# syoyo/lucille

Measured on AMD Instinct MI355X. Metric: Mrays/s (primary+AO), higher is better.
Workload: dtype f32 filter + f64 resolve (hit records f64); 1 GPU; S-soup-1M ray dump (BASELINE config 3): 1000000 random triangles, one dump of 100000000 incoherent rays cut into 1 contiguous slice(s), closest-hit; rays=100000000, rays_per_gpu=100000000, triangles=1000000, mode=closest, variant=-1, parallelism=replicated BVH, ray slices x1

## Files before the change

### include/lucille_hip.h

```cpp
#ifndef LUCILLE_HIP_H
#define LUCILLE_HIP_H

#include <stddef.h>
#include <stdint.h>

#ifdef __cplusplus
extern "C" {
#endif

#define LH_MISS      0xFFFFFFFFu
#define LH_INFINITY  1.0e38

#define LH_MODE_CLOSEST 0
#define LH_MODE_ANY     1

#define LH_VARIANT_DEFAULT (-1)

typedef struct lh_accel lh_accel_t;
typedef struct lh_rib_scene lh_rib_scene_t;

typedef struct lh_accel_info {
    uint32_t ntriangles;
    uint32_t nnodes;
    uint32_t nleaves;
// ... 78 lines not shown

int  lh_accel_intersect_device_tmax(lh_accel_t *accel, size_t n_rays, const void *d_org_xyz, const void *d_dir_xyz,
                                    const void *d_tmax, int ray_format, int record_format,
                                    void *d_prim_or_rec16, void *d_t, void *d_u, void *d_v, void *d_occluded, int mode,
                                    const void *d_index, size_t n_index, const void *d_count, void *stream);
int  lh_accel_intersect_host_tmax(lh_accel_t *accel, size_t n, const void *org_xyz, const void *dir_xyz, const void *tmax,
                                  int ray_format, int record_format, void *prim_or_rec16, double *t, double *u, double *v,
                                  uint8_t *occluded, int mode);

int  lh_accel_intersect_device_counted(lh_accel_t *accel, size_t n, const void *d_org_xyz,
                                       const void *d_dir_xyz, void *d_prim, void *d_t,
                                       void *d_u, void *d_v, void *d_occluded, int mode,
                                       int variant, uint64_t counters[4]);
uint64_t lh_accel_last_retraced(const lh_accel_t *accel);
int lh_accel_dump_node_bytes(const lh_accel_t *accel);

int  lh_accel_trace_statistics(lh_accel_t *accel, int enable);
int  lh_accel_statistics(lh_accel_t *accel, uint64_t counters[5], int clear);
int  lh_accel_slot_statistics(lh_accel_t *accel, uint64_t slots[3], int clear);

int  lh_accel_set_grid(lh_accel_t *accel, int blocks);
int  lh_accel_set_param(lh_accel_t *accel, const char *name, int value);


typedef struct lh_camera {
    int    width, height;
    int    rh;
    int    ortho;
    double flength;
    double cam2world[16];
// ... 215 lines not shown
```

### lucille_amd/binding.py

```python
import atexit
import ctypes as C
import os
import subprocess
import weakref

import numpy as np

HERE = os.path.dirname(os.path.abspath(__file__))
CSRC = os.path.join(HERE, "csrc")

MISS = 0xFFFFFFFF
T_INF = 1.0e38
MODE_CLOSEST, MODE_ANY = 0, 1
VARIANT_DEFAULT, VARIANT_DIRECT, VARIANT_SPEC = -1, 0, 4
RAYS_F64, RAYS_F32 = 0, 1
REC_F64, REC16 = 0, 1
SELECT_HIT, SELECT_MISS, SELECT_OCCLUDED, SELECT_UNOCCLUDED = 0, 1, 2, 3
POS_F64, POS_F32 = 0, 1
AO_NO_HIT = 0xFFFFFFFF


class LucilleHipError(RuntimeError):
    pass

# ... 66 lines not shown


class DirtParams(C.Structure):
    _fields_ = [("near_clip", C.c_double), ("far_clip", C.c_double), ("eps", C.c_double)]

    def __init__(self, near_clip=0.1, far_clip=0.5, eps=1.0e-5):
        super().__init__(float(near_clip), float(far_clip), float(eps))


BEAM_SET_DTYPE = np.dtype([("org", np.float64, (3,)), ("dir", np.float64, (4, 3)), ("normal", np.float64, (4, 3)),
                           ("dominant_axis", np.int32), ("dirsign", np.int32, (3,))])

ABI_SYMBOLS = [
    "lh_device_count", "lh_last_error", "lh_accel_create", "lh_accel_add_mesh", "lh_accel_add_mesh_device", "lh_accel_commit", "lh_accel_wait_exact", "lh_accel_ref_tree",
    "lh_accel_destroy", "lh_accel_info", "lh_accel_prim_lookup", "lh_accel_intersect1", "lh_accel_combine_statistics", "lh_accel_intersect_diag_host", "lh_accel_intersect_diag_device",
    "lh_accel_intersect_host", "lh_accel_intersect_device", "lh_accel_intersect_host_ex", "lh_accel_intersect_device_ex", "lh_accel_intersect_device_indexed", "lh_accel_intersect_device_tmax", "lh_accel_intersect_host_tmax", "lh_accel_compact_device", "lh_accel_intersect_device_counted", "lh_accel_last_retraced", "lh_accel_dump_node_bytes",
    "lh_accel_set_grid", "lh_accel_set_param", "lh_accel_export", "lh_accel_set_normals", "lh_render_primary_rays",
    "lh_render_ao_tile", "lh_render_ao_tile_host", "lh_render_ao_bands", "lh_render_scratch", "lh_accel_beam_visibility_host", "lh_accel_beam_visibility_device", "lh_accel_beam_visibility_set_host", "lh_accel_beam_raster_host", "lh_accel_beam_raster_device", "lh_accel_beam_raster_set_host", "lh_render_pt_tile",
    "lh_accel_trace_statistics", "lh_accel_statistics", "lh_accel_slot_statistics",
    "lh_render_ao_frame_host", "lh_rib_load", "lh_rib_free", "lh_rib_last_error", "lh_rib_info", "lh_rib_messages",
    "lh_rib_mesh", "lh_accel_add_rib_scene", "lh_hdr_write",
    "lh_accel_set_material", "lh_accel_set_environment", "lh_render_pt_tile2", "lh_render_pt_bands", "lh_accel_set_attribute", "lh_accel_set_normals_device", "lh_accel_set_attribute_device",
    "lh_accel_state_build_device", "lh_accel_state_build_host", "lh_accel_ao_device", "lh_accel_ao_host", "lh_accel_ao_rays_device",
    "lh_accel_dirt_device", "lh_accel_dirt_host", "lh_render_dirt_tile",
    "lh_multi_create", "lh_multi_destroy", "lh_multi_ndevices", "lh_multi_accel", "lh_multi_add_mesh", "lh_multi_set_normals",
    "lh_multi_add_rib_scene", "lh_multi_commit", "lh_multi_set_material", "lh_multi_set_environment", "lh_multi_intersect_host",
    "lh_multi_render_ao_frame_host", "lh_multi_render_pt_frame_host",
    "lh_synth_soup_triangles", "lh_synth_soup_rays", "lh_synth_tessellate", "lh_synth_skip",
    "lh_dist_unique_id", "lh_dist_init", "lh_dist_init_file", "lh_dist_destroy", "lh_dist_rank", "lh_dist_world", "lh_dist_transport",
    "lh_dist_barrier", "lh_dist_host_barrier", "lh_dist_broadcast", "lh_dist_gather", "lh_dist_pack_records16", "lh_dist_broadcast_scene", "lh_dist_render_ao_frame_host",
]
# ... 28 lines not shown
    L.lh_accel_destroy.restype = None
    L.lh_accel_info.argtypes = [vp, C.POINTER(AccelInfo)]
    L.lh_accel_prim_lookup.argtypes = [vp, u32, C.POINTER(u32), C.POINTER(u32)]
    L.lh_accel_intersect1.argtypes = [vp, vp, vp, C.POINTER(u32), C.POINTER(C.c_double),
                                      C.POINTER(C.c_double), C.POINTER(C.c_double)]
    L.lh_accel_intersect_host.argtypes = [vp, sz, vp, vp, vp, vp, vp, vp, vp, i32]
    L.lh_accel_intersect_device.argtypes = [vp, sz, vp, vp, vp, vp, vp, vp, vp, i32, i32, vp]
    L.lh_accel_intersect_host_ex.argtypes = [vp, sz, vp, vp, i32, i32, vp, vp, vp, vp, vp, i32]
    L.lh_accel_intersect_device_ex.argtypes = [vp, sz, vp, vp, i32, i32, vp, vp, vp, vp, vp, i32, vp]
    L.lh_accel_intersect_device_indexed.argtypes = [vp, sz, vp, vp, i32, i32, vp, vp, vp, vp, vp, i32, vp, sz, vp, vp]
    L.lh_accel_compact_device.argtypes = [sz, i32, vp, vp, i32, vp, sz, vp, vp, vp, vp]
    L.lh_accel_intersect_device_tmax.argtypes = [vp, sz, vp, vp, vp, i32, i32, vp, vp, vp, vp, vp, i32, vp, sz, vp, vp]
    L.lh_accel_intersect_host_tmax.argtypes = [vp, sz, vp, vp, vp, i32, i32, vp, vp, vp, vp, vp, i32]
    L.lh_accel_last_retraced.argtypes = [vp]; L.lh_accel_last_retraced.restype = C.c_uint64
    L.lh_accel_dump_node_bytes.argtypes = [vp]
    L.lh_accel_intersect_device_counted.argtypes = [vp, sz, vp, vp, vp, vp, vp, vp, vp, i32, i32,
                                                    C.POINTER(C.c_uint64)]
    L.lh_accel_set_grid.argtypes = [vp, i32]
    L.lh_accel_set_param.argtypes = [vp, C.c_char_p, i32]
    L.lh_accel_trace_statistics.argtypes = [vp, i32]
    L.lh_accel_statistics.argtypes = [vp, C.POINTER(C.c_uint64), i32]
    L.lh_accel_slot_statistics.argtypes = [vp, C.POINTER(C.c_uint64), i32]
    L.lh_accel_export.argtypes = [vp, vp, vp]
    L.lh_accel_set_normals.argtypes = [vp, u32, vp, sz, i32]
    L.lh_accel_set_normals_device.argtypes = [vp, u32, u32, vp, i32, sz, i32, vp]
    L.lh_accel_set_attribute_device.argtypes = [vp, u32, i32, u32, vp, i32, sz, vp]
    L.lh_render_primary_rays.argtypes = [vp, C.POINTER(Camera), i32, i32, i32, i32, i32, vp, vp, vp]
    L.lh_render_ao_tile.argtypes = [vp, C.POINTER(Camera), i32, i32, i32, i32, i32, i32, C.c_uint64, vp, vp,
                                    C.POINTER(TileStats), vp]
    L.lh_render_ao_bands.argtypes = [vp, C.POINTER(Camera), i32, C.POINTER(i32), i32, i32, i32, C.c_uint64, vp, C.POINTER(TileStats), vp]
# ... 425 lines not shown
        return out

    def trace_statistics(self, enable=True):
        _check(self.L.lh_accel_trace_statistics(self.h, 1 if enable else 0), "lh_accel_trace_statistics")

    def statistics(self, clear=False):
        c = (C.c_uint64 * 5)()
        _check(self.L.lh_accel_statistics(self.h, c, 1 if clear else 0), "lh_accel_statistics")
        return dict(zip(("nodes", "tris", "exact", "rays", "hits"), (int(x) for x in c)))

    def slot_statistics(self, clear=False):
        c = (C.c_uint64 * 3)()
        _check(self.L.lh_accel_slot_statistics(self.h, c, 1 if clear else 0), "lh_accel_slot_statistics")
        return dict(zip(("node_slots", "tri_slots", "regroups"), (int(x) for x in c)))

    def dump_node_bytes(self):
        return int(self.L.lh_accel_dump_node_bytes(self.h))

    def beam_raster(self, org, corner_dirs, corners, width, height, frame, eye, fov, t_init=None):
        o = np.ascontiguousarray(org, np.float64).reshape(-1, 3); n = o.shape[0]
        d = np.ascontiguousarray(corner_dirs, np.float64).reshape(n, 4, 3)
        c = np.ascontiguousarray(corners, np.float64).reshape(n, 3)
        pl = RasterPlane(int(width), int(height), (C.c_double * 9)(*np.asarray(frame, np.float64).reshape(-1)),
                         (C.c_double * 3)(*np.asarray(eye, np.float64).reshape(-1)), float(fov))
        t = np.zeros((n, height, width)) if t_init is None else np.ascontiguousarray(t_init, np.float64).reshape(n, height, width).copy()
        st = np.empty(n, np.int32); fl = np.zeros((n, 4), np.uint64)
        _check(self.L.lh_accel_beam_raster_host(self.h, n, o.ctypes.data, d.ctypes.data, c.ctypes.data, C.addressof(pl),
                                                t.ctypes.data, st.ctypes.data, fl.ctypes.data), "lh_accel_beam_raster_host")
        return t, st, fl

# ... 475 lines not shown
```

### lucille_amd/csrc/lh_commit.hip

```cpp
#include <assert.h>
#include <thread>
#include <vector>

#include "lh_internal.h"
#include "lh_danger.h"

static thread_local char g_err[512] = "";

extern "C" void lh_set_error(const char *msg) { snprintf(g_err, sizeof(g_err), "%s", msg ? msg : ""); }

int lh_fail(const char *fmt, ...)
{
    va_list ap; va_start(ap, fmt); vsnprintf(g_err, sizeof(g_err), fmt, ap); va_end(ap);
    return -1;
}

pthread_mutex_t g_scene_mu = PTHREAD_MUTEX_INITIALIZER;

extern "C" const char *lh_last_error(void) { return g_err; }

extern "C" int lh_device_count(void)
{
    int n = 0;
    if (hipGetDeviceCount(&n) != hipSuccess) return 0;
// ... 34 lines not shown
    if (env && atoi(env) > 0 && atoi(env) <= 64) { a->tri_batch = atoi(env); a->knobs_user = 1; }
    env = getenv("LH_MIN_ACTIVE");
    if (env && atoi(env) > 0 && atoi(env) <= 64) { a->min_active = atoi(env); a->knobs_user = 1; }
    a->ray_chunk = 256;
    env = getenv("LH_RAY_CHUNK");
    if (env && atoi(env) > 0 && atoi(env) <= (1 << 20)) a->ray_chunk = (uint32_t)atoi(env);
    a->dev.ray_chunk = a->ray_chunk;
    a->dev.ray_budget = LH_RAY_BUDGET; a->dump_budget = LH_DUMP_BUDGET;
    a->ao_budget = LH_AO_BUDGET;
    env = getenv("LH_AO_BUDGET");
    if (env && atoi(env) > 0) { a->ao_budget = (uint32_t)atoi(env); a->ao_budget_user = 1; }
    env = getenv("LH_DUMP_BUDGET");
    if (env && atoi(env) > 0) a->dump_budget = (uint32_t)atoi(env);
    env = getenv("LH_RAY_BUDGET");
    if (env && atoi(env) > 0) a->dev.ray_budget = (uint32_t)atoi(env);
    a->dev.top_nodes = LH_TOP_AUTO;
    a->dev.deg_dcap = INFINITY; a->dev.cap_srcs = 0u; a->dev.ndanger = LH_DANGER_ALL;
    a->dev.coop_patience = 0;
    a->dev.ao_group = 0;
    env = getenv("LH_AO_GROUP");
    if (env && atoi(env) >= 0 && atoi(env) <= 4096) a->dev.ao_group = (uint32_t)atoi(env);
    env = getenv("LH_TOP_NODES");
    if (env && atoi(env) >= 0 && atoi(env) <= (int)LH_TOP_NODES_MAX) a->dev.top_nodes = (uint32_t)atoi(env);
    *out = a;
    return 0;
}

extern "C" int lh_accel_add_mesh(lh_accel_t *a, uint32_t npos, const double *pos, size_t stride,
                                 uint32_t nidx, const uint32_t *idx)
{
// ... 403 lines not shown
    a->d_prim_mesh = a->d_materials = a->d_env_map = NULL;
    free_buf(&a->r_state); free_buf(&a->r_uni); free_buf(&a->r_bands); free_buf(&a->r_diag);
    if (a->h_read) { (void)hipHostFree(a->h_read); a->h_read = NULL; }
    a->d_total = NULL;
    if (a->d_danger) (void)hipFree(a->d_danger);
    a->d_danger = NULL; a->dev.ndanger = LH_DANGER_ALL;
    if (a->d_cursor) (void)hipFree(a->d_cursor);
    if (a->d_counters) (void)hipFree(a->d_counters);
    for (int k = 0; k < LH_AOQ_SLOTS; k++) {
        lh_fixq_t *q = &a->aoq[k].q;
        if (q->queue) {
            (void)hipFree(q->queue); (void)hipFree(q->qcount);
            (void)hipStreamDestroy((hipStream_t)q->aux_stream); (void)hipEventDestroy((hipEvent_t)q->ev_ready); (void)hipEventDestroy((hipEvent_t)q->ev_done);
        }
        memset(q, 0, sizeof(*q)); a->aoq[k].used = 0;
    }
    if (a->pipe.ready) {
        for (int b = 0; b < a->pipe.depth; b++) {
            (void)hipHostFree(a->pipe.h_in[b]); (void)hipHostFree(a->pipe.h_out[b]);
            (void)hipFree(a->pipe.d_in[b]); (void)hipFree(a->pipe.d_out[b]);
            (void)hipEventDestroy(a->pipe.in_done[b]); (void)hipEventDestroy(a->pipe.done[b]);
        }
        for (int b = 0; b < 3; b++) (void)hipStreamDestroy(a->pipe.s[b]);
        a->pipe.ready = 0;
    }
    if (a->d_stage) (void)hipFree(a->d_stage);
    if (a->stream) (void)hipStreamDestroy(a->stream);
    a->d_cursor = a->d_counters = NULL;
    a->d_stage = NULL; a->stage_bytes = 0; a->stream = NULL;
}
// ... 650 lines not shown
    else if (!strcmp(name, "min_active") && value > 0 && value <= 64) { a->min_active = value; a->knobs_user = 1; }
    else if (!strcmp(name, "tri_batch") && value > 0 && value <= 64) { a->tri_batch = value; a->knobs_user = 1; }
    else if (!strcmp(name, "ray_chunk") && value > 0 && value <= (1 << 20)) { a->ray_chunk = (uint32_t)value; a->dev.ray_chunk = (uint32_t)value; }
    else if (!strcmp(name, "variant") && (value == LH_VARIANT_DIRECT || value == LH_VARIANT_SPEC)) a->default_variant = value;
    else if (!strcmp(name, "ray_budget") && value > 0) { a->dev.ray_budget = (uint32_t)value; a->dump_budget = (uint32_t)value; a->ao_budget = (uint32_t)value; a->ao_budget_user = 1; }
    else if (!strcmp(name, "dump_budget") && value > 0) a->dump_budget = (uint32_t)value;
    else if (!strcmp(name, "ao_budget") && value >= 0) { a->ao_budget = (uint32_t)value; a->ao_budget_user = 1; }
    else if (!strcmp(name, "coop_patience") && value >= 0) a->dev.coop_patience = (uint32_t)value;
    else if (!strcmp(name, "ao_fused")) a->ao_fused = value != 0;
    else if (!strcmp(name, "combine")) a->combine = value != 0;
    else if (!strcmp(name, "host_walk")) { a->host_walk = value != 0; a->hw_gpu_left = 0; a->hw_ns = 0.0; }
    else if (!strcmp(name, "ao_group") && value >= 0 && value <= 4096) a->dev.ao_group = (uint32_t)value;
    else if (!strcmp(name, "fast_start")) a->fast_start = value != 0;
    else if (!strcmp(name, "wide8") && value >= -1 && value <= 1) a->wide8 = value;
    else if (!strcmp(name, "top_nodes") && value >= -1 && value <= (int)LH_TOP_NODES_MAX) a->dev.top_nodes = value < 0 ? LH_TOP_AUTO : (uint32_t)value;
    else if (!strcmp(name, "stack_cap") && (value == 0 || (value >= 8 && value <= 64 && value % 2 == 0))) a->dev.stack_cap = (uint32_t)value;
    else return fail("lh_accel_set_param: unknown parameter or bad value: %s = %d", name, value);
    return 0;
}

extern "C" int lh_accel_export(const lh_accel_t *a, void *nodes, void *tri32)
{
    if (!a || !a->committed) return fail("lh_accel_export: accel not committed");
    if (a->hs->device_meshes) return fail("lh_accel_export: the scene was committed from device meshes; there is no host copy");
    if (a->hs->device_built) return fail("lh_accel_export: the tree was built on the device; there is no host copy");
    if (nodes && a->hs->bvh.nnodes) memcpy(nodes, a->hs->bvh.nodes, sizeof(lh_node_t) * (size_t)a->hs->bvh.nnodes);
    if (tri32 && a->hs->bvh.ntris) memcpy(tri32, a->hs->bvh.tri32, sizeof(lh_tri32_t) * (size_t)a->hs->bvh.ntris);
    return 0;
}

// ... 93 lines not shown
```

### lucille_amd/csrc/lh_internal.h

```cpp
#ifndef LH_INTERNAL_H
#define LH_INTERNAL_H

#include <hip/hip_runtime.h>

#include <math.h>
#include <pthread.h>
#include <stdarg.h>
#include <stdio.h>
#include <stdlib.h>
#include <string.h>
#include <time.h>
#include <unistd.h>

#include "../../include/lucille_hip.h"
#include "lh_bvh.h"
#include "lh_refbvh.h"
#include "lh_device.h"

int lh_fail(const char *fmt, ...);
#define fail lh_fail
#define HIPCHK(x) do { hipError_t e_ = (x); if (e_ != hipSuccess) \
    return lh_fail("%s failed: %s", #x, hipGetErrorString(e_)); } while (0)

struct lh_mesh_copy { uint32_t npos, nidx; double *pos; uint32_t *idx; double *nrm; int two_side;
                      double *attr[5]; };

struct lh_dmesh_attr { void *block; size_t stride; int fmt, has; };
#define LH_DATTR_NORMAL 5
#define LH_DATTR_SLOTS 6
struct lh_dmesh { void *block; const void *pos; const uint32_t *idx; size_t stride; uint32_t npos, ntris; int fmt;
                  uint32_t nidx; int two_side; lh_dmesh_attr attr[LH_DATTR_SLOTS]; };
typedef struct lh_dmesh_desc { const void *pos; const uint32_t *idx; unsigned long long stride; uint32_t npos, fmt; } lh_dmesh_desc_t;
// ... 45 lines not shown
    unsigned cursor_next;
    pthread_mutex_t mu;
    int stat_on;
    unsigned long long stat[5];
    unsigned long long stat_slots[3];
    hipStream_t stream;
    uint64_t device_bytes;
    double upload_seconds;
    int grid_blocks;
    int grid_user;
    int min_active;
    uint32_t ray_chunk;
    int tri_batch;
    int knobs_user;
    int default_variant;
    struct { hipStream_t stream; int used; lh_fixq_t q; } aoq[LH_AOQ_SLOTS];
    void *d_stage; size_t stage_bytes;
    struct { void *h_in[LH_PIPE_DEPTH_MAX], *h_out[LH_PIPE_DEPTH_MAX], *d_in[LH_PIPE_DEPTH_MAX], *d_out[LH_PIPE_DEPTH_MAX]; hipStream_t s[3];
             hipEvent_t in_done[LH_PIPE_DEPTH_MAX], done[LH_PIPE_DEPTH_MAX]; size_t cap; int depth, ready; } pipe;
    void *d_nrm9;
    void *d_attr9[3], *d_st6, *d_inside;
    void *d_prim_mesh;
    lh_material_t *materials; uint32_t nmaterials; void *d_materials; int materials_dirty;
    lh_environment_t env; void *d_env_map; int env_set;
    lh_buf r_state;
    lh_buf r_uni;
    lh_buf r_diag;
    lh_buf r_bands;
    void *h_read;
    lh_buf r_org, r_dir, r_prim, r_t, r_u, r_v, r_frame;
    lh_ao_scratch tile_ao;
    lh_ao_scratch batch_ao;
    lh_buf b_tot, b_host;
    lh_ao_scratch tile_dirt, batch_dirt;
    lh_dirt_scratch tile_dirt_t, batch_dirt_t;
    lh_buf d_tot, d_rays;
    uint64_t last_retraced;
    int ao_fused;
    uint32_t ao_budget;
    int ao_budget_user;
    uint32_t dump_budget;
    int build_auto;
    int poison_outputs;
    int fast_start;
    lh_buf p_org2, p_dir2, p_path, p_path2, p_thr, p_thr2, p_rad, p_counts;
    unsigned long long *d_total;
    size_t r_nsamples, r_nslots, r_nao;
    struct lh_combiner *comb;
    int combine;
    int host_walk; unsigned long long hw_calls; double hw_ns; int hw_gpu_left;
};

#define LH_NCURSOR 64

struct lh_guard {
    pthread_mutex_t *m;
// ... 43 lines not shown
struct lh_launch_opt {
    uint32_t io_fmt = 0u;
    uint32_t *diag_out = NULL;
    const uint32_t *n_dev = NULL;
    const void *cam_src = NULL;
    unsigned long long *diag_clock = NULL;
    bool indexed = false; const uint32_t *index = NULL; uint32_t idx_nrays = 0u;
    const void *tmax = NULL;
};
int  lh_launch(lh_accel_t *a, const lh_batch_t &batch, int variant, hipStream_t s, bool dump, const lh_launch_opt &opt = lh_launch_opt());
static inline unsigned long long *lh_next_cursor(lh_accel_t *a)
{
    return (unsigned long long *)((uint32_t *)a->d_cursor + (size_t)LH_CURSOR_WORDS * (a->cursor_next++ % LH_NCURSOR));
}
int  lh_aoq_slot(lh_accel_t *a, hipStream_t s);
static inline void lh_stat_add(lh_accel_t *a, const unsigned long long *h, unsigned long long rays, unsigned long long hits, bool slots = false)
{
    a->stat[0] += h[LH_CNT_NODES]; a->stat[1] += h[LH_CNT_TRIS]; a->stat[2] += h[LH_CNT_EXACT];
    a->stat[3] += rays; a->stat[4] += hits;
    if (slots) { a->stat_slots[0] += h[LH_CNT_NODE_SLOTS]; a->stat_slots[1] += h[LH_CNT_TRI_SLOTS]; a->stat_slots[2] += h[LH_CNT_REGROUP_SLOTS]; }
}
int  lh_ensure_stage(lh_accel_t *a, size_t bytes);

extern "C" int lh_render_launch_primary(const lh_camera_t *cam, int x0, int y0, int w, int h, int xs, int ys,
                                        double *d_org, double *d_dir, void *stream);
extern "C" int lh_render_launch_compact(const lh_dev_scene_t *sc, const double *d_nrm9, size_t n, const double *d_org,
                                        const double *d_dir, const uint32_t *d_prim, const double *d_t,
                                        const double *d_u, const double *d_v, uint32_t *d_block_counts,
                                        uint32_t *d_slot_of_sample, double *d_hitrec,
                                        unsigned long long *d_slot_key, int x0, int w, int nbands, int band_rows,
// ... 50 lines not shown
```

### lucille_amd/csrc/lh_query.hip

```cpp
#include <atomic>
#include <chrono>
#include <condition_variable>
#include <deque>
#include <mutex>
#include <thread>
#include <vector>

#include "lh_internal.h"

__global__ void k_fill_listed(size_t n, const uint32_t *index, const uint32_t *count, uint32_t nrays, int miss,
                              uint32_t *prim, double *t, double *u, double *v, uint8_t *occ, uint4 *rec16, unsigned long long *counters)
{
    const size_t k = (size_t)blockIdx.x * blockDim.x + threadIdx.x;
    if (count && *count < n) n = *count;
    if (k >= n) return;
    const uint32_t i = index ? index[k] : (uint32_t)k;
    if (i >= nrays) return;
    const uint32_t w = miss ? LH_MISS_PRIM : 0x77777777u;
    const unsigned long long d = 0x7777777777777777ull;
    if (rec16) { uint4 r; r.x = w; r.y = miss ? __float_as_uint((float)LH_T_INF) : w; r.z = r.w = miss ? __float_as_uint(0.0f) : w; rec16[i] = r; }
    if (prim) prim[i] = w;
    if (t) t[i] = miss ? LH_T_INF : __longlong_as_double((long long)d);
    if (u) u[i] = miss ? 0.0 : __longlong_as_double((long long)d);
    if (v) v[i] = miss ? 0.0 : __longlong_as_double((long long)d);
// ... 58 lines not shown

static bool dump_walks_q8(const lh_accel_t *a, int variant)
{
    return variant == LH_VARIANT_SPEC && q8_available(a) && (a->wide8 == 1 || (a->wide8 == -1 && wide8_pays(a)));
}

static int batch_args(const lh_accel_t *a, const char *what, size_t n, bool have_arrays, const char *arrays, int mode)
{
    if (!a || !a->committed) return fail("%s: accel not committed", what);
    if (n == 0) return 0;
    if (!have_arrays) return fail("%s: NULL %s", what, arrays);
    if (mode != LH_MODE_CLOSEST && mode != LH_MODE_ANY) return fail("%s: unknown mode %d", what, mode);
    return 1;
}

int lh_launch(lh_accel_t *a, const lh_batch_t &b, int variant, hipStream_t s, bool dump, const lh_launch_opt &opt)
{
    const int go = batch_args(a, "intersect", b.n, (b.org && b.dir) || opt.cam_src, "ray arrays", b.mode);
    if (go <= 0) return go;
    const size_t n = b.n;
    const bool closest = b.mode == LH_MODE_CLOSEST, rec16 = closest && (opt.io_fmt & LH_IO_REC16);
    if (rec16 && (!b.prim || b.t || b.u || b.v)) return fail("intersect: 16-byte records go to one array (t, u, v must be NULL)");
    if (closest && !rec16 && (!b.prim || !b.t || !b.u || !b.v)) return fail("intersect: closest mode needs prim,t,u,v outputs");
    if (!closest && !b.occ) return fail("intersect: any mode needs the occluded output");
    HIPCHK(hipSetDevice(a->device));
    const bool miss = a->hs->bvh.ntris == 0;
    if (miss || (opt.indexed && dump && a->poison_outputs)) {
        const size_t step = (size_t)1 << 30;
        for (size_t off = 0; off < n; off += step) {
            const lh_batch_t f = lh_batch_sub(b, opt.io_fmt, off, n - off < step ? n - off : step);
// ... 23 lines not shown
    const bool q8 = dump && dump_walks_q8(a, variant);
    if (q8 && lh_ensure_formats(a, LH_FMT_Q8) != 0) return -1;
    const int qk = lh_aoq_slot(a, s);
    if (qk < 0) return -1;
    lh_dev_scene_t sc = a->dev;
    sc.prefer_q8 = q8;
    if (dump) sc.ray_budget = a->dump_budget;
    else if (sc.ray_chunk < LH_TILE_CHUNK) sc.ray_chunk = LH_TILE_CHUNK;
    sc.io_fmt = opt.io_fmt & (closest ? (LH_IO_RAYS_F32 | LH_IO_REC16) : LH_IO_RAYS_F32);
    sc.diag_out = opt.diag_out; sc.n_dev = opt.n_dev; sc.cam_src = opt.cam_src; sc.diag_clock = opt.diag_clock;
    sc.index = opt.indexed ? opt.index : NULL; sc.idx_nrays = opt.indexed ? opt.idx_nrays : 0u;
    if (opt.tmax && (!opt.indexed || !dump || variant != LH_VARIANT_SPEC)) return fail("intersect: per-ray bounds are read by the default walk's indexed ray dumps only");
    sc.tmax = opt.tmax;
    const bool dump4 = dump && !q8 && !a->knobs_user;
    const bool dump8 = dump && q8 && !a->knobs_user;
    const int rc = lh_launch_trace(&sc, &b, lh_next_cursor(a), variant, a->grid_blocks,
                                   dump4 ? LH_DUMP_MIN_ACTIVE : dump8 ? LH_DUMP8_MIN_ACTIVE : a->min_active, dump4 ? LH_DUMP_TRI_BATCH : dump8 ? LH_DUMP8_TRI_BATCH : a->tri_batch,
                                   &a->aoq[qk].q, a->ncus, (void *)s);
    if (rc != 0) return fail("kernel launch failed: %s", hipGetErrorString(hipGetLastError()));
    return 0;
}

extern "C" int lh_accel_intersect_device(lh_accel_t *a, size_t n, const void *d_org, const void *d_dir,
                                         void *d_prim, void *d_t, void *d_u, void *d_v, void *d_occ,
                                         int mode, int variant, void *stream)
{
    lh_guard guard(a);
    return lh_launch(a, lh_batch_t{n, mode, d_org, d_dir, d_prim, d_t, d_u, d_v, d_occ, NULL}, variant, (hipStream_t)stream, true);
}

static int counted_begin(lh_accel_t *a, hipStream_t s) { HIPCHK(hipMemsetAsync(a->d_counters, 0, sizeof(unsigned long long) * LH_CNT_DEV, s)); return 0; }
static int counted_collect(lh_accel_t *a, hipStream_t s, unsigned long long h[LH_CNT_DEV])
{
// ... 23 lines not shown
    for (int k = 0; k < LH_CNT_N; k++) counters[k] = h[k];
    if (getenv("LH_DEBUG_COUNTERS"))
        fprintf(stderr, "[lucille_hip] lane slots: node steps %llu of %llu, triangle steps %llu of %llu, regroup iterations %llu; "
                        "rays through the reference walk %llu\n",
                h[LH_CNT_NODES], h[LH_CNT_NODE_SLOTS], h[LH_CNT_TRIS], h[LH_CNT_TRI_SLOTS], h[LH_CNT_REGROUP_SLOTS], h[LH_CNT_RETRACED]);
    return 0;
}

extern "C" int lh_accel_dump_node_bytes(const lh_accel_t *a)
{
    if (!a || !a->committed || a->hs->bvh.ntris == 0) return 0;
    return dump_walks_q8(a, a->default_variant) ? (int)sizeof(lh_q8node_t) : 64;
}

extern "C" uint64_t lh_accel_last_retraced(const lh_accel_t *a) { return a ? a->last_retraced : 0; }

int lh_ensure_stage(lh_accel_t *a, size_t bytes)
{
    if (a->stage_bytes >= bytes) return 0;
    if (a->d_stage) { (void)hipFree(a->d_stage); a->d_stage = NULL; a->stage_bytes = 0; }
    HIPCHK(hipMalloc(&a->d_stage, bytes));
    a->stage_bytes = bytes;
    return 0;
}

#define LH_PIPE_CHUNK_DEFAULT ((size_t)1 << 21)
#define LH_PIPE_DEPTH_DEFAULT 3
#define LH_PIPE_MIN   ((size_t)1 << 21)
#define LH_COPY_SLICE ((size_t)1 << 20)

// ... 765 lines not shown
```

Measured before the change: 2311 Mrays/s.

## Sort large incoherent ray dumps by origin cell before tracing, scatter results back

Adds a device-side counting sort that bins rays by a coarse Morton cell of their origin (optionally by direction octant), copies them into a reordered workspace, traces the reordered batch, and scatters hit records back to the original order. It targets the divergence and poor cache reuse of BVH traversal over incoherent ray dumps, enabled by default for large dumps on the default walk. In exchange it adds extra passes over the ray and result arrays and a large workspace allocation, which could cost more than the coherence gain on random rays against a random triangle soup.

After: 2494 Mrays/s (median of 6 runs). 7.9% higher.

```diff
diff --git a/include/lucille_hip.h b/include/lucille_hip.h
--- a/include/lucille_hip.h
+++ b/include/lucille_hip.h
@@ -116,6 +116,7 @@
                                        int variant, uint64_t counters[4]);
 uint64_t lh_accel_last_retraced(const lh_accel_t *accel);
 int lh_accel_dump_node_bytes(const lh_accel_t *accel);
+int lh_accel_order_statistics(lh_accel_t *accel, uint64_t out[2], int clear);
 
 int  lh_accel_trace_statistics(lh_accel_t *accel, int enable);
 int  lh_accel_statistics(lh_accel_t *accel, uint64_t counters[5], int clear);
diff --git a/lucille_amd/binding.py b/lucille_amd/binding.py
--- a/lucille_amd/binding.py
+++ b/lucille_amd/binding.py
@@ -104,7 +104,7 @@
 ABI_SYMBOLS = [
     "lh_device_count", "lh_last_error", "lh_accel_create", "lh_accel_add_mesh", "lh_accel_add_mesh_device", "lh_accel_commit", "lh_accel_wait_exact", "lh_accel_ref_tree",
     "lh_accel_destroy", "lh_accel_info", "lh_accel_prim_lookup", "lh_accel_intersect1", "lh_accel_combine_statistics", "lh_accel_intersect_diag_host", "lh_accel_intersect_diag_device",
-    "lh_accel_intersect_host", "lh_accel_intersect_device", "lh_accel_intersect_host_ex", "lh_accel_intersect_device_ex", "lh_accel_intersect_device_indexed", "lh_accel_intersect_device_tmax", "lh_accel_intersect_host_tmax", "lh_accel_compact_device", "lh_accel_intersect_device_counted", "lh_accel_last_retraced", "lh_accel_dump_node_bytes",
+    "lh_accel_intersect_host", "lh_accel_intersect_device", "lh_accel_intersect_host_ex", "lh_accel_intersect_device_ex", "lh_accel_intersect_device_indexed", "lh_accel_intersect_device_tmax", "lh_accel_intersect_host_tmax", "lh_accel_compact_device", "lh_accel_intersect_device_counted", "lh_accel_last_retraced", "lh_accel_dump_node_bytes", "lh_accel_order_statistics",
     "lh_accel_set_grid", "lh_accel_set_param", "lh_accel_export", "lh_accel_set_normals", "lh_render_primary_rays",
     "lh_render_ao_tile", "lh_render_ao_tile_host", "lh_render_ao_bands", "lh_render_scratch", "lh_accel_beam_visibility_host", "lh_accel_beam_visibility_device", "lh_accel_beam_visibility_set_host", "lh_accel_beam_raster_host", "lh_accel_beam_raster_device", "lh_accel_beam_raster_set_host", "lh_render_pt_tile",
     "lh_accel_trace_statistics", "lh_accel_statistics", "lh_accel_slot_statistics",
@@ -163,6 +163,8 @@
     L.lh_accel_intersect_host_tmax.argtypes = [vp, sz, vp, vp, vp, i32, i32, vp, vp, vp, vp, vp, i32]
     L.lh_accel_last_retraced.argtypes = [vp]; L.lh_accel_last_retraced.restype = C.c_uint64
     L.lh_accel_dump_node_bytes.argtypes = [vp]
+    if hasattr(L, "lh_accel_order_statistics"):
+        L.lh_accel_order_statistics.argtypes = [vp, C.POINTER(C.c_uint64), i32]
     L.lh_accel_intersect_device_counted.argtypes = [vp, sz, vp, vp, vp, vp, vp, vp, vp, i32, i32,
                                                     C.POINTER(C.c_uint64)]
     L.lh_accel_set_grid.argtypes = [vp, i32]
@@ -618,6 +620,11 @@
         _check(self.L.lh_accel_slot_statistics(self.h, c, 1 if clear else 0), "lh_accel_slot_statistics")
         return dict(zip(("node_slots", "tri_slots", "regroups"), (int(x) for x in c)))
 
+    def order_statistics(self, clear=False):
+        c = (C.c_uint64 * 2)()
+        _check(self.L.lh_accel_order_statistics(self.h, c, 1 if clear else 0), "lh_accel_order_statistics")
+        return {"dumps": int(c[0]), "rays": int(c[1])}
+
     def dump_node_bytes(self):
         return int(self.L.lh_accel_dump_node_bytes(self.h))
 
diff --git a/lucille_amd/csrc/lh_commit.hip b/lucille_amd/csrc/lh_commit.hip
--- a/lucille_amd/csrc/lh_commit.hip
+++ b/lucille_amd/csrc/lh_commit.hip
@@ -72,6 +72,9 @@
     if (env && atoi(env) > 0) a->dump_budget = (uint32_t)atoi(env);
     env = getenv("LH_RAY_BUDGET");
     if (env && atoi(env) > 0) a->dev.ray_budget = (uint32_t)atoi(env);
+    a->dump_order = 1; a->dump_order_min = LH_DUMP_ORDER_MIN; a->dump_order_bits = LH_DUMP_ORDER_BITS; a->dump_order_max_mb = 0;
+    env = getenv("LH_DUMP_ORDER");
+    if (env) a->dump_order = atoi(env) != 0;
     a->dev.top_nodes = LH_TOP_AUTO;
     a->dev.deg_dcap = INFINITY; a->dev.cap_srcs = 0u; a->dev.ndanger = LH_DANGER_ALL;
     a->dev.coop_patience = 0;
@@ -505,6 +508,7 @@
             (void)hipStreamDestroy((hipStream_t)q->aux_stream); (void)hipEventDestroy((hipEvent_t)q->ev_ready); (void)hipEventDestroy((hipEvent_t)q->ev_done);
         }
         memset(q, 0, sizeof(*q)); a->aoq[k].used = 0;
+        free_buf(&a->aoq[k].order_ws);
     }
     if (a->pipe.ready) {
         for (int b = 0; b < a->pipe.depth; b++) {
@@ -1185,6 +1189,10 @@
     else if (!strcmp(name, "fast_start")) a->fast_start = value != 0;
     else if (!strcmp(name, "wide8") && value >= -1 && value <= 1) a->wide8 = value;
     else if (!strcmp(name, "top_nodes") && value >= -1 && value <= (int)LH_TOP_NODES_MAX) a->dev.top_nodes = value < 0 ? LH_TOP_AUTO : (uint32_t)value;
+    else if (!strcmp(name, "dump_order")) a->dump_order = value != 0;
+    else if (!strcmp(name, "dump_order_min") && value > 0) a->dump_order_min = (size_t)value;
+    else if (!strcmp(name, "dump_order_bits") && (value == 1 || value == 2)) a->dump_order_bits = (uint32_t)value;
+    else if (!strcmp(name, "dump_order_max_mb") && value >= 0) a->dump_order_max_mb = (size_t)value;
     else if (!strcmp(name, "stack_cap") && (value == 0 || (value >= 8 && value <= 64 && value % 2 == 0))) a->dev.stack_cap = (uint32_t)value;
     else return fail("lh_accel_set_param: unknown parameter or bad value: %s = %d", name, value);
     return 0;
diff --git a/lucille_amd/csrc/lh_internal.h b/lucille_amd/csrc/lh_internal.h
--- a/lucille_amd/csrc/lh_internal.h
+++ b/lucille_amd/csrc/lh_internal.h
@@ -16,6 +16,7 @@
 #include "lh_bvh.h"
 #include "lh_refbvh.h"
 #include "lh_device.h"
+#include "lh_order.h"
 
 int lh_fail(const char *fmt, ...);
 #define fail lh_fail
@@ -91,7 +92,7 @@
     int tri_batch;
     int knobs_user;
     int default_variant;
-    struct { hipStream_t stream; int used; lh_fixq_t q; } aoq[LH_AOQ_SLOTS];
+    struct { hipStream_t stream; int used; lh_fixq_t q; lh_buf order_ws; } aoq[LH_AOQ_SLOTS];
     void *d_stage; size_t stage_bytes;
     struct { void *h_in[LH_PIPE_DEPTH_MAX], *h_out[LH_PIPE_DEPTH_MAX], *d_in[LH_PIPE_DEPTH_MAX], *d_out[LH_PIPE_DEPTH_MAX]; hipStream_t s[3];
              hipEvent_t in_done[LH_PIPE_DEPTH_MAX], done[LH_PIPE_DEPTH_MAX]; size_t cap; int depth, ready; } pipe;
@@ -117,6 +118,8 @@
     uint32_t ao_budget;
     int ao_budget_user;
     uint32_t dump_budget;
+    int dump_order; size_t dump_order_min; uint32_t dump_order_bits; size_t dump_order_max_mb;
+    unsigned long long order_stat[2];
     int build_auto;
     int poison_outputs;
     int fast_start;
@@ -190,6 +193,8 @@
     return (unsigned long long *)((uint32_t *)a->d_cursor + (size_t)LH_CURSOR_WORDS * (a->cursor_next++ % LH_NCURSOR));
 }
 int  lh_aoq_slot(lh_accel_t *a, hipStream_t s);
+int  lh_order_run(const lh_order_plan_t *p, const lh_order_grid_t *g, const void *d_org, const void *d_dir, void *d_ws, hipStream_t stream);
+int  lh_order_back(const lh_order_plan_t *p, int closest, const void *d_ws, void *d_prim, void *d_t, void *d_u, void *d_v, void *d_occ, hipStream_t stream);
 static inline void lh_stat_add(lh_accel_t *a, const unsigned long long *h, unsigned long long rays, unsigned long long hits, bool slots = false)
 {
     a->stat[0] += h[LH_CNT_NODES]; a->stat[1] += h[LH_CNT_TRIS]; a->stat[2] += h[LH_CNT_EXACT];
diff --git a/lucille_amd/csrc/lh_order.h b/lucille_amd/csrc/lh_order.h
--- /dev/null
+++ b/lucille_amd/csrc/lh_order.h
@@ -0,0 +1,129 @@
+#ifndef LH_ORDER_H
+#define LH_ORDER_H
+
+#include <stdint.h>
+#include <stddef.h>
+#include <string.h>
+
+#if defined(__HIPCC__)
+#define LH_ORDER_FN static inline __host__ __device__
+#else
+#define LH_ORDER_FN static inline
+#endif
+
+#define LH_ORDER_BLOCK     4096u
+#define LH_ORDER_MIN_RUN   48u
+#define LH_DUMP_ORDER_BITS 2u
+#define LH_DUMP_ORDER_MIN  ((size_t)16000000)
+#define LH_ORDER_ALIGN     256u
+
+typedef struct lh_order_grid { double lo[3], scale[3]; uint32_t bits, octant; } lh_order_grid_t;
+
+LH_ORDER_FN lh_order_grid_t lh_order_grid(const float grid_lo[3], const float grid_step[3], uint32_t bits, uint32_t octant)
+{
+    lh_order_grid_t g; int k;
+    g.bits = bits; g.octant = octant ? 1u : 0u;
+    for (k = 0; k < 3; k++) { g.lo[k] = (double)grid_lo[k]; g.scale[k] = (double)(1u << bits) / (65535.0 * (double)grid_step[k]); }
+    return g;
+}
+
+LH_ORDER_FN uint32_t lh_order_keybits(uint32_t bits, uint32_t octant) { return 3u * bits + (octant ? 3u : 0u); }
+LH_ORDER_FN int      lh_order_valid(uint32_t bits, uint32_t octant) { const uint32_t kb = lh_order_keybits(bits, octant); return kb == 3u || kb == 6u || kb == 9u; }
+LH_ORDER_FN uint32_t lh_order_nbins(uint32_t bits, uint32_t octant) { return 1u << lh_order_keybits(bits, octant); }
+
+LH_ORDER_FN uint32_t lh_order_block(uint32_t bits, uint32_t octant)
+{
+    uint32_t b = LH_ORDER_BLOCK;
+    while (b < LH_ORDER_MIN_RUN * lh_order_nbins(bits, octant)) b *= 2u;
+    return b;
+}
+
+LH_ORDER_FN uint32_t lh_order_cell(double x, double lo, double scale, uint32_t bits)
+{
+    const double f = (x - lo) * scale, top = (double)(1u << bits);
+    if (!(f >= 0.0)) return 0u;
+    if (f >= top) return (1u << bits) - 1u;
+    return (uint32_t)f;
+}
+
+LH_ORDER_FN uint32_t lh_order_sign(double x)
+{
+    uint64_t w;
+    memcpy(&w, &x, sizeof(w));
+    return (uint32_t)(w >> 63);
+}
+
+LH_ORDER_FN uint32_t lh_order_key(const double org[3], const double dir[3], const lh_order_grid_t *g)
+{
+    const uint32_t cx = lh_order_cell(org[0], g->lo[0], g->scale[0], g->bits);
+    const uint32_t cy = lh_order_cell(org[1], g->lo[1], g->scale[1], g->bits);
+    const uint32_t cz = lh_order_cell(org[2], g->lo[2], g->scale[2], g->bits);
+    const uint32_t octant = lh_order_sign(dir[0]) | (lh_order_sign(dir[1]) << 1) | (lh_order_sign(dir[2]) << 2);
+    uint32_t m = 0u, b;
+    for (b = 0; b < g->bits; b++)
+        m |= (((cx >> b) & 1u) << (3u * b)) | (((cy >> b) & 1u) << (3u * b + 1u)) | (((cz >> b) & 1u) << (3u * b + 2u));
+    return g->octant ? (octant << (3u * g->bits)) | m : m;
+}
+
+typedef struct lh_order_plan {
+    size_t   n;
+    uint32_t bits, octant, nbins, block, nblocks;
+    size_t   org, dir, t, u, v, prim, occ, dest, slot, counts, offset, bintotal, binbase;
+    size_t   bytes;
+} lh_order_plan_t;
+
+LH_ORDER_FN size_t lh_order_up(size_t x) { return (x + (LH_ORDER_ALIGN - 1u)) & ~(size_t)(LH_ORDER_ALIGN - 1u); }
+
+LH_ORDER_FN lh_order_plan_t lh_order_plan(size_t n, uint32_t bits, uint32_t octant, int closest)
+{
+    lh_order_plan_t p; size_t at = 0, table;
+    p.n = n; p.bits = bits; p.octant = octant ? 1u : 0u; p.nbins = lh_order_nbins(bits, octant); p.block = lh_order_block(bits, octant);
+    p.nblocks = (uint32_t)((n + p.block - 1u) / p.block);
+    table = (size_t)p.nblocks * p.nbins * sizeof(uint32_t);
+    p.org = at; at = lh_order_up(at + n * 24u);
+    p.dir = at; at = lh_order_up(at + n * 24u);
+    p.t = p.u = p.v = p.prim = p.occ = at;
+    if (closest) {
+        p.t = at; at = lh_order_up(at + n * 8u);
+        p.u = at; at = lh_order_up(at + n * 8u);
+        p.v = at; at = lh_order_up(at + n * 8u);
+        p.prim = at; at = lh_order_up(at + n * 4u);
+    } else {
+        p.occ = at; at = lh_order_up(at + n);
+    }
+    p.dest = at; at = lh_order_up(at + n * 4u);
+    p.slot = at; at = lh_order_up(at + n * 2u);
+    p.counts = at; at = lh_order_up(at + table);
+    p.offset = at; at = lh_order_up(at + table);
+    p.bintotal = at; at = lh_order_up(at + p.nbins * sizeof(uint32_t));
+    p.binbase = at; at = lh_order_up(at + p.nbins * sizeof(uint32_t));
+    p.bytes = at;
+    return p;
+}
+
+LH_ORDER_FN void lh_order_offsets(const uint32_t *counts, uint32_t nblocks, uint32_t nbins, uint32_t *offset)
+{
+    uint32_t run = 0u, k, b;
+    for (k = 0; k < nbins; k++)
+        for (b = 0; b < nblocks; b++) { offset[(size_t)b * nbins + k] = run; run += counts[(size_t)b * nbins + k]; }
+}
+
+#if !defined(__HIPCC__)
+LH_ORDER_FN void lh_order_host(size_t n, const double *org, const double *dir, const lh_order_grid_t *g, uint32_t *key, uint32_t *counts,
+                               uint32_t *offset, uint32_t *dest)
+{
+    const uint32_t nbins = lh_order_nbins(g->bits, g->octant), block = lh_order_block(g->bits, g->octant), nblocks = (uint32_t)((n + block - 1u) / block);
+    size_t i;
+    memset(counts, 0, (size_t)nblocks * nbins * sizeof(uint32_t));
+    for (i = 0; i < n; i++) {
+        const uint32_t k = lh_order_key(org + 3 * i, dir + 3 * i, g);
+        if (key) key[i] = k;
+        counts[(i / block) * nbins + k]++;
+    }
+    lh_order_offsets(counts, nblocks, nbins, offset);
+    for (i = 0; i < n; i++) dest[i] = offset[(i / block) * nbins + lh_order_key(org + 3 * i, dir + 3 * i, g)]++;
+    for (i = 0; i < (size_t)nblocks * nbins; i++) offset[i] -= counts[i];
+}
+#endif
+
+#endif
diff --git a/lucille_amd/csrc/lh_order.hip b/lucille_amd/csrc/lh_order.hip
--- /dev/null
+++ b/lucille_amd/csrc/lh_order.hip
@@ -0,0 +1,243 @@
+#include "lh_internal.h"
+#include "lh_order.h"
+
+#define ORD_T      256
+#define ORD_NB     64u
+#define ORD_TILE   1024u
+#define ORD_PER    (ORD_TILE / ORD_T)
+#define ORD_SLICES (ORD_TILE / 64u)
+#define ORD_CHUNKS (ORD_T * 48 / 16)
+
+struct OrdRays { const char *org, *dir; size_t n; lh_order_grid_t g; };
+
+__device__ __forceinline__ uint4 ord_load16(const char *base, size_t off, size_t nbytes)
+{
+    uint4 r = make_uint4(0u, 0u, 0u, 0u);
+    if (off + 16 <= nbytes) r = *(const uint4 *)(base + off);
+    else if (off + 8 <= nbytes) { const uint2 h = *(const uint2 *)(base + off); r.x = h.x; r.y = h.y; }
+    return r;
+}
+
+template <bool OCT>
+__global__ __launch_bounds__(ORD_T) void k_order_count(OrdRays a, uint32_t *counts)
+{
+    constexpr uint32_t STEP = OCT ? ORD_T : 2 * ORD_T;
+    __shared__ uint4 stage[2][ORD_CHUNKS];
+    __shared__ uint32_t hist[ORD_NB];
+    const size_t first = (size_t)blockIdx.x * LH_ORDER_BLOCK, nbytes = a.n * 24u;
+    const size_t m = a.n - first < LH_ORDER_BLOCK ? a.n - first : LH_ORDER_BLOCK;
+    const uint32_t nstep = (uint32_t)((m + STEP - 1) / STEP);
+    uint4 v[3];
+    auto fetch = [&](size_t r0) {
+#pragma unroll
+        for (int j = 0; j < 3; j++) {
+            const uint32_t q = threadIdx.x + ORD_T * j;
+            const bool o = !OCT || q < ORD_CHUNKS / 2;
+            v[j] = ord_load16(o ? a.org : a.dir, r0 * 24u + (size_t)(o ? q : q - ORD_CHUNKS / 2) * 16u, nbytes);
+        }
+    };
+    if (threadIdx.x < ORD_NB) hist[threadIdx.x] = 0u;
+    fetch(first);
+#pragma unroll
+    for (int j = 0; j < 3; j++) stage[0][threadIdx.x + ORD_T * j] = v[j];
+    __syncthreads();
+    for (uint32_t p = 0; p < nstep; p++) {
+        const bool more = p + 1 < nstep;
+        if (more) fetch(first + (size_t)(p + 1) * STEP);
+        const double *so = (const double *)stage[p & 1];
+        if (OCT) {
+            const double *sd = so + 3 * ORD_T;
+            if ((size_t)p * STEP + threadIdx.x < m) atomicAdd(&hist[lh_order_key(so + 3 * threadIdx.x, sd + 3 * threadIdx.x, &a.g)], 1u);
+        } else {
+#pragma unroll
+            for (uint32_t h = 0; h < 2; h++) {
+                const uint32_t i = threadIdx.x + ORD_T * h;
+                if ((size_t)p * STEP + i < m) atomicAdd(&hist[lh_order_key(so + 3 * i, so + 3 * i, &a.g)], 1u);
+            }
+        }
+        if (more) {
+#pragma unroll
+            for (int j = 0; j < 3; j++) stage[(p + 1) & 1][threadIdx.x + ORD_T * j] = v[j];
+        }
+        __syncthreads();
+    }
+    if (threadIdx.x < ORD_NB) counts[(size_t)blockIdx.x * ORD_NB + threadIdx.x] = hist[threadIdx.x];
+}
+
+__device__ __forceinline__ uint32_t ord_block_scan(uint32_t x, uint32_t *lds, uint32_t *total)
+{
+    const uint32_t t = threadIdx.x, nt = blockDim.x;
+    uint32_t incl = x;
+    lds[t] = x;
+    __syncthreads();
+    for (uint32_t s = 1; s < nt; s *= 2) {
+        const uint32_t y = t >= s ? lds[t - s] : 0u;
+        __syncthreads();
+        incl += y; lds[t] = incl;
+        __syncthreads();
+    }
+    *total = lds[nt - 1];
+    return incl - x;
+}
+
+__global__ __launch_bounds__(ORD_T) void k_order_scan_blocks(const uint32_t *counts, uint32_t *offset, uint32_t *bintotal, uint32_t nblocks)
+{
+    __shared__ uint32_t lds[ORD_T];
+    const uint32_t bin = blockIdx.x, per = (nblocks + ORD_T - 1) / ORD_T;
+    const uint32_t lo = threadIdx.x * per < nblocks ? threadIdx.x * per : nblocks, hi = lo + per < nblocks ? lo + per : nblocks;
+    uint32_t sum = 0u, total;
+    for (uint32_t b = lo; b < hi; b++) sum += counts[(size_t)b * ORD_NB + bin];
+    uint32_t run = ord_block_scan(sum, lds, &total);
+    for (uint32_t b = lo; b < hi; b++) { offset[(size_t)b * ORD_NB + bin] = run; run += counts[(size_t)b * ORD_NB + bin]; }
+    if (threadIdx.x == 0) bintotal[bin] = total;
+}
+
+__global__ void k_order_scan_bins(const uint32_t *bintotal, uint32_t *binbase)
+{
+    __shared__ uint32_t lds[ORD_NB];
+    uint32_t total;
+    binbase[threadIdx.x] = ord_block_scan(bintotal[threadIdx.x], lds, &total);
+}
+
+__global__ __launch_bounds__(ORD_T) void k_order_copy(OrdRays a, const uint32_t *offset, const uint32_t *binbase, double *oorg, double *odir, uint32_t *dest, uint16_t *slots)
+{
+    __shared__ double img[2][ORD_TILE * 3];
+    __shared__ uint32_t cnt[ORD_SLICES][ORD_NB], sdest[ORD_TILE];
+    __shared__ uint32_t start[ORD_NB], gbase[ORD_NB], base[ORD_NB];
+    const size_t first = (size_t)blockIdx.x * LH_ORDER_BLOCK;
+    const size_t m = a.n - first < LH_ORDER_BLOCK ? a.n - first : LH_ORDER_BLOCK;
+    const uint32_t ntiles = (uint32_t)((m + ORD_TILE - 1) / ORD_TILE);
+    const uint32_t lane = threadIdx.x & 63u, w = threadIdx.x >> 6;
+    const double *org = (const double *)a.org, *dir = (const double *)a.dir;
+    double o[ORD_PER][3], d[ORD_PER][3];
+    auto fetch = [&](size_t tile0, uint32_t mt) {
+#pragma unroll
+        for (uint32_t s = 0; s < ORD_PER; s++) {
+            const uint32_t j = s * ORD_T + threadIdx.x;
+            const size_t r = 3 * (tile0 + (j < mt ? j : 0u));
+#pragma unroll
+            for (int c = 0; c < 3; c++) { o[s][c] = org[r + c]; d[s][c] = dir[r + c]; }
+        }
+    };
+    if (w == 0) base[lane] = binbase[lane] + offset[(size_t)blockIdx.x * ORD_NB + lane];
+    fetch(first, (uint32_t)(m < ORD_TILE ? m : ORD_TILE));
+    for (uint32_t tile = 0; tile < ntiles; tile++) {
+        const size_t tile0 = first + (size_t)tile * ORD_TILE;
+        const uint32_t mt = (uint32_t)(first + m - tile0 < ORD_TILE ? first + m - tile0 : ORD_TILE);
+        uint32_t key[ORD_PER], rank[ORD_PER];
+#pragma unroll
+        for (uint32_t s = 0; s < ORD_PER; s++) {
+            const bool valid = s * ORD_T + threadIdx.x < mt;
+            key[s] = valid ? lh_order_key(o[s], d[s], &a.g) : 0u;
+            unsigned long long mine = __ballot(valid), have = mine;
+#pragma unroll
+            for (uint32_t i = 0; i < 6; i++) {
+                const unsigned long long b = __ballot((key[s] >> i) & 1u);
+                mine &= ((key[s] >> i) & 1u) ? b : ~b;
+                have &= ((lane >> i) & 1u) ? b : ~b;
+            }
+            rank[s] = __popcll(mine & ((1ull << lane) - 1ull));
+            cnt[s * (ORD_T / 64) + w][lane] = __popcll(have);
+        }
+        __syncthreads();
+        if (w == 0) {
+            uint32_t run = 0u;
+            for (uint32_t q = 0; q < ORD_SLICES; q++) { const uint32_t c = cnt[q][lane]; cnt[q][lane] = run; run += c; }
+            uint32_t incl = run;
+#pragma unroll
+            for (uint32_t s = 1; s < 64; s *= 2) { const uint32_t y = __shfl_up(incl, s); if (lane >= s) incl += y; }
+            start[lane] = incl - run; gbase[lane] = base[lane]; base[lane] += run;
+        }
+        __syncthreads();
+#pragma unroll
+        for (uint32_t s = 0; s < ORD_PER; s++) {
+            const uint32_t j = s * ORD_T + threadIdx.x;
+            if (j < mt) {
+                const uint32_t p = cnt[s * (ORD_T / 64) + w][key[s]] + rank[s], slot = start[key[s]] + p, at = gbase[key[s]] + p;
+#pragma unroll
+                for (int c = 0; c < 3; c++) { img[0][3 * slot + c] = o[s][c]; img[1][3 * slot + c] = d[s][c]; }
+                sdest[slot] = at; dest[tile0 + j] = at; slots[tile0 + j] = (uint16_t)slot;
+            }
+        }
+        if (tile + 1 < ntiles) fetch(tile0 + ORD_TILE, (uint32_t)(first + m - tile0 - ORD_TILE < ORD_TILE ? first + m - tile0 - ORD_TILE : ORD_TILE));
+        __syncthreads();
+        for (uint32_t e = threadIdx.x; e < 3 * mt; e += ORD_T) {
+            const uint32_t slot = e / 3u, at = sdest[slot];
+            if (at < a.n) {
+                const size_t g = 3 * (size_t)at + (e - 3u * slot);
+                oorg[g] = img[0][e]; odir[g] = img[1][e];
+            }
+        }
+    }
+}
+
+template <bool CLOSEST>
+__global__ __launch_bounds__(ORD_T) void k_order_back(size_t n, const uint32_t *dest, const uint16_t *slots, const uint32_t *sprim, const double *st, const double *su,
+                                                      const double *sv, const uint8_t *socc, uint32_t *prim, double *t, double *u, double *v, uint8_t *occ)
+{
+    __shared__ uint32_t sdest[ORD_TILE];
+    __shared__ uint16_t sray[ORD_TILE];
+    __shared__ double bt[CLOSEST ? ORD_TILE : 1], bu[CLOSEST ? ORD_TILE : 1], bv[CLOSEST ? ORD_TILE : 1];
+    __shared__ uint32_t bp[CLOSEST ? ORD_TILE : 1];
+    __shared__ uint8_t bo[CLOSEST ? 1 : ORD_TILE];
+    const size_t first = (size_t)blockIdx.x * LH_ORDER_BLOCK;
+    const size_t m = n - first < LH_ORDER_BLOCK ? n - first : LH_ORDER_BLOCK;
+    const uint32_t ntiles = (uint32_t)((m + ORD_TILE - 1) / ORD_TILE);
+    for (uint32_t tile = 0; tile < ntiles; tile++) {
+        const size_t tile0 = first + (size_t)tile * ORD_TILE;
+        const uint32_t mt = (uint32_t)(first + m - tile0 < ORD_TILE ? first + m - tile0 : ORD_TILE);
+#pragma unroll
+        for (uint32_t s = 0; s < ORD_PER; s++) {
+            const uint32_t j = s * ORD_T + threadIdx.x;
+            if (j < mt) { const uint32_t slot = slots[tile0 + j] & (ORD_TILE - 1u); sdest[slot] = dest[tile0 + j]; sray[slot] = (uint16_t)j; }
+        }
+        __syncthreads();
+#pragma unroll
+        for (uint32_t s = 0; s < ORD_PER; s++) {
+            const uint32_t j = s * ORD_T + threadIdx.x;
+            if (j < mt) {
+                const uint32_t at = sdest[j] < n ? sdest[j] : 0u, i = sray[j] & (ORD_TILE - 1u);
+                if (CLOSEST) { bp[i] = sprim[at]; bt[i] = st[at]; bu[i] = su[at]; bv[i] = sv[at]; }
+                else bo[i] = socc[at];
+            }
+        }
+        __syncthreads();
+#pragma unroll
+        for (uint32_t s = 0; s < ORD_PER; s++) {
+            const uint32_t j = s * ORD_T + threadIdx.x;
+            if (j < mt) {
+                if (CLOSEST) { prim[tile0 + j] = bp[j]; t[tile0 + j] = bt[j]; u[tile0 + j] = bu[j]; v[tile0 + j] = bv[j]; }
+                else occ[tile0 + j] = bo[j];
+            }
+        }
+    }
+}
+
+int lh_order_run(const lh_order_plan_t *p, const lh_order_grid_t *g, const void *d_org, const void *d_dir, void *d_ws, hipStream_t stream)
+{
+    if (!p || p->n == 0 || p->n > ((size_t)1 << 30) || p->nbins != ORD_NB || p->block != LH_ORDER_BLOCK || (((uintptr_t)d_org | (uintptr_t)d_dir) & 15u)) return -1;
+    char *ws = (char *)d_ws;
+    const OrdRays a = {(const char *)d_org, (const char *)d_dir, p->n, *g};
+    uint32_t *counts = (uint32_t *)(ws + p->counts), *offset = (uint32_t *)(ws + p->offset), *bintotal = (uint32_t *)(ws + p->bintotal), *binbase = (uint32_t *)(ws + p->binbase);
+    if (g->octant) hipLaunchKernelGGL(k_order_count<true>, dim3(p->nblocks), dim3(ORD_T), 0, stream, a, counts);
+    else hipLaunchKernelGGL(k_order_count<false>, dim3(p->nblocks), dim3(ORD_T), 0, stream, a, counts);
+    hipLaunchKernelGGL(k_order_scan_blocks, dim3(ORD_NB), dim3(ORD_T), 0, stream, counts, offset, bintotal, p->nblocks);
+    hipLaunchKernelGGL(k_order_scan_bins, dim3(1), dim3(ORD_NB), 0, stream, bintotal, binbase);
+    hipLaunchKernelGGL(k_order_copy, dim3(p->nblocks), dim3(ORD_T), 0, stream, a, offset, binbase, (double *)(ws + p->org), (double *)(ws + p->dir), (uint32_t *)(ws + p->dest),
+                       (uint16_t *)(ws + p->slot));
+    return hipGetLastError() == hipSuccess ? 0 : -1;
+}
+
+int lh_order_back(const lh_order_plan_t *p, int closest, const void *d_ws, void *d_prim, void *d_t, void *d_u, void *d_v, void *d_occ, hipStream_t stream)
+{
+    const char *ws = (const char *)d_ws;
+    const uint32_t *dest = (const uint32_t *)(ws + p->dest);
+    const uint16_t *slots = (const uint16_t *)(ws + p->slot);
+    if (closest)
+        hipLaunchKernelGGL(k_order_back<true>, dim3(p->nblocks), dim3(ORD_T), 0, stream, p->n, dest, slots, (const uint32_t *)(ws + p->prim), (const double *)(ws + p->t),
+                           (const double *)(ws + p->u), (const double *)(ws + p->v), (const uint8_t *)NULL, (uint32_t *)d_prim, (double *)d_t, (double *)d_u, (double *)d_v, (uint8_t *)NULL);
+    else
+        hipLaunchKernelGGL(k_order_back<false>, dim3(p->nblocks), dim3(ORD_T), 0, stream, p->n, dest, slots, (const uint32_t *)NULL, (const double *)NULL, (const double *)NULL,
+                           (const double *)NULL, (const uint8_t *)(ws + p->occ), (uint32_t *)NULL, (double *)NULL, (double *)NULL, (double *)NULL, (uint8_t *)d_occ);
+    return hipGetLastError() == hipSuccess ? 0 : -1;
+}
diff --git a/lucille_amd/csrc/lh_query.hip b/lucille_amd/csrc/lh_query.hip
--- a/lucille_amd/csrc/lh_query.hip
+++ b/lucille_amd/csrc/lh_query.hip
@@ -96,6 +96,17 @@
     return 1;
 }
 
+static void *order_workspace(lh_accel_t *a, int qk, const lh_order_plan_t &p)
+{
+    lh_buf *w = &a->aoq[qk].order_ws;
+    if (a->dump_order_max_mb && p.bytes > (a->dump_order_max_mb << 20)) return NULL;
+    if (w->p && w->cap >= p.bytes) return w->p;
+    lh_free_buf(w);
+    if (hipMalloc(&w->p, p.bytes) != hipSuccess) { (void)hipGetLastError(); w->p = NULL; return NULL; }
+    w->cap = p.bytes;
+    return w->p;
+}
+
 int lh_launch(lh_accel_t *a, const lh_batch_t &b, int variant, hipStream_t s, bool dump, const lh_launch_opt &opt)
 {
     const int go = batch_args(a, "intersect", b.n, (b.org && b.dir) || opt.cam_src, "ray arrays", b.mode);
@@ -149,9 +160,29 @@
     sc.tmax = opt.tmax;
     const bool dump4 = dump && !q8 && !a->knobs_user;
     const bool dump8 = dump && q8 && !a->knobs_user;
-    const int rc = lh_launch_trace(&sc, &b, lh_next_cursor(a), variant, a->grid_blocks,
-                                   dump4 ? LH_DUMP_MIN_ACTIVE : dump8 ? LH_DUMP8_MIN_ACTIVE : a->min_active, dump4 ? LH_DUMP_TRI_BATCH : dump8 ? LH_DUMP8_TRI_BATCH : a->tri_batch,
-                                   &a->aoq[qk].q, a->ncus, (void *)s);
+    const int min_active = dump4 ? LH_DUMP_MIN_ACTIVE : dump8 ? LH_DUMP8_MIN_ACTIVE : a->min_active, tri_batch = dump4 ? LH_DUMP_TRI_BATCH : dump8 ? LH_DUMP8_TRI_BATCH : a->tri_batch;
+    const bool ordered = dump && a->dump_order && n >= a->dump_order_min && variant == LH_VARIANT_SPEC && sc.io_fmt == 0u && !opt.indexed && !opt.tmax &&
+                         !opt.cam_src && !opt.n_dev && !opt.diag_out && !opt.diag_clock && !(((uintptr_t)b.org | (uintptr_t)b.dir) & 15u);
+    if (ordered) {
+        const size_t step = (size_t)1 << 30;
+        const uint32_t octant = a->dump_order_bits == 1u;
+        char *ws = (char *)order_workspace(a, qk, lh_order_plan(n < step ? n : step, a->dump_order_bits, octant, closest));
+        const lh_order_grid_t g = lh_order_grid(sc.grid_lo, sc.grid_step, a->dump_order_bits, octant);
+        for (size_t off = 0; ws && off < n; off += step) {
+            const lh_batch_t part = lh_batch_sub(b, 0u, off, n - off < step ? n - off : step);
+            const lh_order_plan_t p = lh_order_plan(part.n, a->dump_order_bits, octant, closest);
+            if (a->poison_outputs) HIPCHK(hipMemsetAsync(ws + (closest ? p.t : p.occ), 0x77, p.dest - (closest ? p.t : p.occ), s));
+            if (lh_order_run(&p, &g, part.org, part.dir, ws, s) != 0) return fail("ordering a ray dump failed: %s", hipGetErrorString(hipGetLastError()));
+            const lh_batch_t o = {part.n, b.mode, ws + p.org, ws + p.dir, closest ? ws + p.prim : NULL, closest ? ws + p.t : NULL, closest ? ws + p.u : NULL,
+                                  closest ? ws + p.v : NULL, closest ? NULL : ws + p.occ, b.counters};
+            if (lh_launch_trace(&sc, &o, lh_next_cursor(a), variant, a->grid_blocks, min_active, tri_batch, &a->aoq[qk].q, a->ncus, (void *)s) != 0 ||
+                lh_order_back(&p, closest ? 1 : 0, ws, part.prim, part.t, part.u, part.v, part.occ, s) != 0)
+                return fail("kernel launch failed: %s", hipGetErrorString(hipGetLastError()));
+            a->order_stat[0]++; a->order_stat[1] += part.n;
+        }
+        if (ws) return 0;
+    }
+    const int rc = lh_launch_trace(&sc, &b, lh_next_cursor(a), variant, a->grid_blocks, min_active, tri_batch, &a->aoq[qk].q, a->ncus, (void *)s);
     if (rc != 0) return fail("kernel launch failed: %s", hipGetErrorString(hipGetLastError()));
     return 0;
 }
@@ -205,6 +236,15 @@
 }
 
 extern "C" uint64_t lh_accel_last_retraced(const lh_accel_t *a) { return a ? a->last_retraced : 0; }
+
+extern "C" int lh_accel_order_statistics(lh_accel_t *a, uint64_t out[2], int clear)
+{
+    lh_guard guard(a);
+    if (!a || !out) return fail("lh_accel_order_statistics: NULL argument");
+    out[0] = a->order_stat[0]; out[1] = a->order_stat[1];
+    if (clear) a->order_stat[0] = a->order_stat[1] = 0;
+    return 0;
+}
 
 int lh_ensure_stage(lh_accel_t *a, size_t bytes)
 {
```
